# AlgoLab/rs-vgaligner

Hardware: AMD Instinct MI355X
Metric: aligned reads/sec (10 kbp ONT vs HLA graph) (higher is better)
Workload: dtype int32+f64

## Files before the change

include/vga_hip.h:

```cpp
#ifndef VGA_HIP_H
#define VGA_HIP_H

#include <stddef.h>
#include <stdint.h>

#ifdef __cplusplus
extern "C" {
#endif

#define VGA_OK 0
#define VGA_ERR_ARG (-1)
#define VGA_ERR_HIP (-2)
#define VGA_ERR_NOMEM (-3)
#define VGA_ERR_UNSUPPORTED (-4)
#define VGA_ERR_NO_INDEX (-5)
#define VGA_ERR_NO_DEVICE (-6)
#define VGA_ERR_POOL (-7)

#define VGA_NO_PRED (-1)

#define VGA_MAX_KMER_LENGTH 32

typedef struct vga_ctx vga_ctx;

// ... 106 lines not shown
    int32_t *best_score;
    uint64_t *path_off;
    uint32_t *abpoa_nodes;
    uint32_t *graph_nodes;
    uint32_t *aln_start_offset;
    uint32_t *aln_end_offset;
    uint32_t *n_aligned_bases;
    uint64_t *cigar_off;
    char *cigar;
    uint64_t *cs_off;
    char *cs;
    uint64_t *n_rows;
    uint64_t *n_cells;
    uint64_t *n_value_cells;
    float ms_dp, ms_traceback, ms_total;
} vga_poa_result;
void vga_poa_result_free(vga_poa_result *r);

int vga_poa_batch(vga_ctx *ctx, uint64_t n, const uint64_t *node_ptr, const uint64_t *node_off,
                  const char *nodes_concat, const uint64_t *edge_ptr, const uint32_t *edge_src,
                  const uint32_t *edge_dst, const uint64_t *query_off, const char *queries_concat,
                  const vga_poa_params *params, vga_poa_result **out);

typedef struct {
    uint64_t n_reads;
    uint8_t *aligned;
    uint64_t *path_off;
    uint64_t *path_handles;
    uint32_t *path_length;
    uint32_t *path_start;
    uint32_t *path_end;
    uint32_t *block_length;
    int32_t *best_score;
    uint64_t *cigar_off;
    char *cigar;
    uint64_t *cs_off;
    char *cs;
    uint64_t poa_rows, poa_cells, poa_value_cells, poa_problems;
    float ms_subgraph, ms_dp, ms_traceback, ms_total;
    uint64_t result_bytes;
} vga_align_result;

int vga_align_batch(vga_batch *b, const vga_map_result *chains, uint32_t align_best_n,
                    const vga_poa_params *params, vga_align_result **out);
void vga_align_result_free(vga_align_result *r);
int vga_align_prepare(vga_ctx *ctx, uint64_t n_reads, uint32_t max_read_len);

int vga_coverage_begin(vga_ctx *ctx);
int vga_coverage_read(vga_ctx *ctx, uint32_t *base_depth , uint32_t *node_reads ,
                      uint32_t *edge_reads , uint64_t *n_alignments);
int vga_coverage_reset(vga_ctx *ctx);
int vga_coverage_end(vga_ctx *ctx);

int vga_path_support_begin(vga_ctx *ctx, uint32_t n_paths, const uint64_t *step_off , const uint64_t *steps,
                           uint64_t *n_pairs_without_edge);
// ... 112 lines not shown
```

rs-vgaligner_amd/binding.py:

```python
from __future__ import annotations

import ctypes as C
import os
from typing import List, Optional, Sequence

import numpy as np

_HERE = os.path.dirname(os.path.abspath(__file__))
LIB_PATH = os.environ.get("VGA_LIB") or os.path.join(_HERE, "libvga_hip.so")

VGA_OK = 0
VGA_MAX_KMER_LENGTH = 32
VGA_STRANDS_FORWARD = 0
VGA_STRANDS_BOTH = 1
ERR_NAMES = {-1: "VGA_ERR_ARG", -2: "VGA_ERR_HIP", -3: "VGA_ERR_NOMEM", -4: "VGA_ERR_UNSUPPORTED",
             -5: "VGA_ERR_NO_INDEX", -6: "VGA_ERR_NO_DEVICE", -7: "VGA_ERR_POOL"}

PILEUP_COLUMNS = ("A", "C", "G", "T", "N", "del", "ins")

ABI_SYMBOLS = [
    "vga_ctx_create", "vga_ctx_destroy", "vga_last_error", "vga_ctx_synchronize", "vga_abi_version",
    "vga_index_upload", "vga_batch_create", "vga_batch_destroy", "vga_batch_strands", "vga_map_default_params", "vga_map_batch",
    "vga_map_result_free", "vga_poa_default_params", "vga_poa_result_free", "vga_poa_batch", "vga_align_batch",
    "vga_align_result_free", "vga_last_kernel_times", "vga_chain_paths_text", "vga_chain_text_free",
# ... 118 lines not shown
        ("max_chain_score", _P(C.c_double)), ("best_pred_id", _P(C.c_int32)), ("curr_max", _P(C.c_double)),
        ("n_chains", C.c_uint64), ("chain_off", _P(C.c_uint64)), ("chain_placeholder", _P(C.c_uint8)),
        ("chain_anchor_off", _P(C.c_uint64)), ("chain_anchor_idx", _P(C.c_uint32)),
        ("ms_probe", C.c_float), ("ms_sort", C.c_float), ("ms_chain", C.c_float), ("ms_total", C.c_float),
        ("n_hits", C.c_uint64), ("strand", _P(C.c_uint8)),
    ]


class PoaResult(C.Structure):
    _fields_ = [
        ("n", C.c_uint64), ("ok", _P(C.c_uint8)), ("best_score", _P(C.c_int32)), ("path_off", _P(C.c_uint64)),
        ("abpoa_nodes", _P(C.c_uint32)), ("graph_nodes", _P(C.c_uint32)), ("aln_start_offset", _P(C.c_uint32)),
        ("aln_end_offset", _P(C.c_uint32)), ("n_aligned_bases", _P(C.c_uint32)), ("cigar_off", _P(C.c_uint64)),
        ("cigar", _P(C.c_char)), ("cs_off", _P(C.c_uint64)), ("cs", _P(C.c_char)), ("n_rows", _P(C.c_uint64)),
        ("n_cells", _P(C.c_uint64)), ("n_value_cells", _P(C.c_uint64)), ("ms_dp", C.c_float), ("ms_traceback", C.c_float), ("ms_total", C.c_float),
    ]


class AlignResult(C.Structure):
    _fields_ = [
        ("n_reads", C.c_uint64), ("aligned", _P(C.c_uint8)), ("path_off", _P(C.c_uint64)), ("path_handles", _P(C.c_uint64)),
        ("path_length", _P(C.c_uint32)), ("path_start", _P(C.c_uint32)), ("path_end", _P(C.c_uint32)),
        ("block_length", _P(C.c_uint32)), ("best_score", _P(C.c_int32)), ("cigar_off", _P(C.c_uint64)),
        ("cigar", _P(C.c_char)), ("cs_off", _P(C.c_uint64)), ("cs", _P(C.c_char)),
        ("poa_rows", C.c_uint64), ("poa_cells", C.c_uint64), ("poa_value_cells", C.c_uint64), ("poa_problems", C.c_uint64),
        ("ms_subgraph", C.c_float), ("ms_dp", C.c_float), ("ms_traceback", C.c_float), ("ms_total", C.c_float),
        ("result_bytes", C.c_uint64),
    ]


class KernelTime(C.Structure):
    _fields_ = [("name", C.c_char_p), ("ms", C.c_float), ("launches", C.c_uint32), ("algorithmic_bytes", C.c_uint64),
                ("busy_ms", C.c_float), ("reserved", C.c_uint32)]


_lib = None


def load_library():
    global _lib
    if _lib is not None:
        return _lib
# ... 344 lines not shown
        tp = int(self.path_off[-1])
        self.abpoa_nodes = _np(r.abpoa_nodes, tp, np.uint32)
        self.graph_nodes = _np(r.graph_nodes, tp, np.uint32)
        self.aln_start_offset = _np(r.aln_start_offset, n, np.uint32)
        self.aln_end_offset = _np(r.aln_end_offset, n, np.uint32)
        self.n_aligned_bases = _np(r.n_aligned_bases, n, np.uint32)
        self.cigar_off = _np(r.cigar_off, n + 1, np.uint64)
        self.cs_off = _np(r.cs_off, n + 1, np.uint64)
        cig = C.string_at(r.cigar, int(self.cigar_off[-1])) if n else b""
        cs = C.string_at(r.cs, int(self.cs_off[-1])) if n else b""
        self.cigar = [cig[int(self.cigar_off[i]):int(self.cigar_off[i + 1]) - 1].decode() for i in range(n)]
        self.cs = [cs[int(self.cs_off[i]):int(self.cs_off[i + 1]) - 1].decode() for i in range(n)]
        self.n_rows = _np(r.n_rows, n, np.uint64)
        self.n_cells = _np(r.n_cells, n, np.uint64)
        self.n_value_cells = _np(r.n_value_cells, n, np.uint64)
        self.ms = {"dp": r.ms_dp, "traceback": r.ms_traceback, "total": r.ms_total}
        L.vga_poa_result_free(ptr)


class AlignOut:
    def __init__(self, L, ptr):
        r = ptr.contents
        R = int(r.n_reads)
        self.n_reads = R
        self.aligned = _np(r.aligned, R, np.uint8)
        self.path_off = _np(r.path_off, R + 1, np.uint64)
        self.path_handles = _np(r.path_handles, int(self.path_off[-1]), np.uint64)
        self.path_length = _np(r.path_length, R, np.uint32)
        self.path_start = _np(r.path_start, R, np.uint32)
        self.path_end = _np(r.path_end, R, np.uint32)
        self.block_length = _np(r.block_length, R, np.uint32)
        self.best_score = _np(r.best_score, R, np.int32)
        self.cigar_off = _np(r.cigar_off, R + 1, np.uint64)
        self.cs_off = _np(r.cs_off, R + 1, np.uint64)
        cig = C.string_at(r.cigar, int(self.cigar_off[-1])) if R else b""
        cs = C.string_at(r.cs, int(self.cs_off[-1])) if R else b""
        self.cigar = [cig[int(self.cigar_off[i]):int(self.cigar_off[i + 1]) - 1].decode() for i in range(R)]
        self.cs = [cs[int(self.cs_off[i]):int(self.cs_off[i + 1]) - 1].decode() for i in range(R)]
        self.poa_rows, self.poa_cells, self.poa_problems = int(r.poa_rows), int(r.poa_cells), int(r.poa_problems)
        self.poa_value_cells = int(r.poa_value_cells)
        self.ms = {"subgraph": r.ms_subgraph, "dp": r.ms_dp, "traceback": r.ms_traceback, "total": r.ms_total}
        L.vga_align_result_free(ptr)


class Batch:
    def __init__(self, ctx: "Context", seqs: Sequence):
        self.ctx = ctx
        L = ctx.L
        self.seqs = list(seqs)
        raw = [s if isinstance(s, (bytes, bytearray)) else s.encode() for s in self.seqs]
        self._concat = b"".join(raw)
        off = np.zeros(len(self.seqs) + 1, dtype=np.uint64)
        if self.seqs:
            off[1:] = np.cumsum([len(s) for s in raw], dtype=np.uint64)
        self._off = off
# ... 57 lines not shown
        t0 = _t.perf_counter()
        self.ctx._check(L.vga_map_batch(self.h, C.byref(mp), C.byref(m)))
        t1 = _t.perf_counter()
        kt_map = self.ctx.kernel_times()
        try:
            a = _P(AlignResult)()
            self.ctx._check(L.vga_align_batch(self.h, m, best_n, C.byref(pp), C.byref(a)))
            self.ctx._last_reads = len(self.seqs)
            t2 = _t.perf_counter()
            kt_aln = self.ctx.kernel_times()
            r, q = a.contents, m.contents
            R = int(r.n_reads)
            aligned = int(np.ctypeslib.as_array(r.aligned, shape=(R,)).sum()) if R else 0
            out = dict(n_reads=R, aligned=aligned, n_anchors=int(q.n_anchors), n_hits=int(q.n_hits),
                       poa_rows=int(r.poa_rows), poa_cells=int(r.poa_cells), poa_value_cells=int(r.poa_value_cells),
                       poa_problems=int(r.poa_problems), path_bases=int(np.ctypeslib.as_array(r.path_length, shape=(R,)).sum()) if R else 0,
                       cigar_bytes=int(r.cigar_off[R]) if R else 0, result_bytes=int(r.result_bytes),
                       ms_map=float(q.ms_total), ms_probe=float(q.ms_probe), ms_sort=float(q.ms_sort), ms_chain=float(q.ms_chain),
                       ms_align=float(r.ms_total), ms_subgraph=float(r.ms_subgraph), ms_dp_summed_launches=float(r.ms_dp),
                       ms_traceback=float(r.ms_traceback), kernels=kt_map + kt_aln)
            if on_results is not None:
                on_results(q, r)
            t3 = _t.perf_counter()
            L.vga_align_result_free(a)
        finally:
            L.vga_map_result_free(m)
        t4 = _t.perf_counter()
        out["ms_wall_map_call"] = (t1 - t0) * 1e3
        out["ms_wall_align_call"] = (t2 - t1) * 1e3
        out["ms_wall_free"] = (t4 - t3) * 1e3
        return out
# ... 529 lines not shown
```

rs-vgaligner_amd/csrc/vga_align.hip:

```cpp
#include "vga_align_plan.hpp"
#include "vga_common.hpp"
#include "vga_coverage.hpp"
#include "vga_path_edit.hpp"
#include "vga_path_support.hpp"
#include "vga_pileup.hpp"
#include "vga_insertion.hpp"
#include "vga_poa_internal.hpp"
#include "vga_subgraph_host.hpp"

#include <algorithm>
#include <atomic>
#include <chrono>
#include <memory>

extern "C" void vga_align_result_free(vga_align_result *r)
{
    if (!r) return;
    free(r->aligned); free(r->path_off); free(r->path_handles); free(r->path_length); free(r->path_start);
    free(r->path_end); free(r->block_length); free(r->best_score); free(r->cigar_off); free(r->cigar);
    free(r->cs_off); free(r->cs);
    free(r);
}

namespace {
// ... 272 lines not shown
        res->path_length[r] = it.n_path;
        res->path_start[r] = it.start_off;
        res->path_end[r] = it.end_off;
        res->block_length[r] = it.aligned;
        res->best_score[r] = it.score;
        if (it.cs_p) {
            memcpy(res->cigar + res->cigar_off[r], it.cigar_p, it.cigar_n); res->cigar[res->cigar_off[r] + it.cigar_n] = 0;
            memcpy(res->cs + res->cs_off[r], it.cs_p, it.cs_n); res->cs[res->cs_off[r] + it.cs_n] = 0;
        } else {
            memcpy(res->cigar + res->cigar_off[r], it.cigar.c_str(), it.cigar.size() + 1);
            memcpy(res->cs + res->cs_off[r], it.cs.c_str(), it.cs.size() + 1);
        }
    });
    res->poa_problems = n;
    for (uint64_t p = 0; p < n; p++) {
        res->poa_rows += items[p].n_rows; res->poa_cells += items[p].n_cells; res->poa_value_cells += items[p].n_vcells;
    }
    res->ms_subgraph = (float)sub_ms;
    res->ms_dp = tm.ms_dp;
    res->ms_traceback = tm.ms_tb;
    res->result_bytes = tm.result_bytes;
    res->ms_total = (float)std::chrono::duration<double, std::milli>(std::chrono::steady_clock::now() - t0).count();
    tr.mark("assemble records");
    if (tr.on && !on_device) sg_host_walk::trace_thread_time();
    return VGA_OK;
}

}

static int vga_align_batch_impl(vga_batch *b, const vga_map_result *m, uint32_t align_best_n, const vga_poa_params *params,
                               vga_align_result **out)
// ... 39 lines not shown
```

rs-vgaligner_amd/csrc/vga_poa_internal.hpp:

```cpp
#pragma once

#include <cstdint>
#include <functional>
#include <string>
#include <vector>

#include "vga_common.hpp"
#include "vga_subgraph.hpp"

struct poa_view {
    const uint64_t *node_off;
    const char *nodes;
    uint64_t n_nodes;
    const uint32_t *esrc, *edst;
    uint64_t n_edges;
    const char *query;
    uint32_t qlen;
};

struct poa_item {
    uint8_t ok = 0;
    int32_t score = 0;
    uint32_t start_off = 0, end_off = 0, aligned = 0;
    uint64_t n_rows = 0, n_cells = 0, n_vcells = 0;
    uint32_t n_path = 0;
    bool deduped = false;
    std::vector<uint32_t> rows;
    std::vector<uint32_t> gnodes;
    std::string cigar, cs;
    const char *cs_p = nullptr, *cigar_p = nullptr;
    const uint32_t *gnodes_p = nullptr;
    uint32_t cs_n = 0, cigar_n = 0, gnodes_n = 0;
};

struct poa_timing {
    float ms_dp = 0, ms_tb = 0, ms_total = 0;
    uint64_t result_bytes = 0;
};

// ... 16 lines not shown
```

rs-vgaligner_amd/csrc/vga_poa_launch.hpp:

```cpp
#pragma once

#include "vga_common.hpp"
#include "vga_poa_shape.hpp"
#include "vga_subgraph.hpp"

#define POA_CHUNK (1ull << 20)
#define POA_RING_SPAN 32
#define POA_SLOTS 4

#define POA_ST_OK 0
#define POA_ST_POOL 1
#define POA_ST_NOALN 2
#define POA_ST_TRACE 3
#define POA_ST_RETRY 5

struct poa_prob {
    uint64_t node0;
    uint64_t pred0;
    uint64_t sink0;
    uint64_t q0;
    uint64_t ops0;
    uint64_t row0;
    uint64_t seq0;
    uint32_t n_sink;
// ... 9 lines not shown
struct poa_row {
    int32_t beg, end;
    uint64_t doff, voff;
    int32_t lmax, rmax;
    uint32_t pred, npred;
    int32_t base, hmax;
};
static_assert(sizeof(poa_row) == 48 && offsetof(poa_row, pred) == 32, "poa_row layout");

struct poa_out {
    int32_t score;
    uint32_t row;
    int32_t status;
    uint32_t maxw;
    uint64_t cells, vcells;
    uint32_t nops, pad;
    uint64_t t_begin, t_end;
};

struct poa_dev_params {
    int32_t match, mismatch, o1, e1, o2, e2, banded;
};

#define POA_NIL 0xFFFFFFFFu
#define POA_LISTS 64
#define POA_LIST_STRIDE 16
struct poa_chunk_pool {
    unsigned long long *head;
    uint32_t *next;
    const uint64_t *seg_base;
    uint32_t cps_log2;
// ... 66 lines not shown
```

rs-vgaligner_amd/csrc/vga_poa_pool.hpp:

```cpp
#pragma once

#include <atomic>
#include <chrono>
#include <condition_variable>
#include <memory>
#include <mutex>
#include <thread>
#include <vector>

#include "vga_common.hpp"
#include "vga_poa_launch.hpp"

struct poa_slot {
    vga_dbuf<poa_prob> d_probs;
    vga_dbuf<uint4> d_ntab;
    vga_dbuf<uint32_t> d_seq32, d_preds, d_sink, d_orow, d_ids;
    vga_dbuf<uint8_t> d_ops;
    vga_dbuf<poa_row> d_rows;
    vga_dbuf<poa_out> d_outs;
    vga_dbuf<char> d_q;
    vga_hbuf<poa_prob> h_probs;
    vga_hbuf<uint4> h_ntab;
    vga_hbuf<uint32_t> h_seq32, h_preds, h_sink, h_ids;
    vga_hbuf<char> h_q;
    vga_dbuf<char> d_text;
    vga_dbuf<poa_text_out> d_touts;
    vga_dbuf<unsigned long long> d_tcur;
    struct out_set {
        vga_hbuf<uint32_t> h_orow;
        vga_hbuf<uint8_t> h_ops;
        vga_hbuf<char> h_seq;
        vga_hbuf<poa_out> h_outs;
        vga_hbuf<char> h_text;
        char *text_p = nullptr;
        vga_hbuf<poa_text_out> h_touts;
        vga_hbuf<unsigned long long> h_tcur;
        bool text = false;
        uint64_t tot_ops = 0, tot_seq = 0;
    } outs[2];
    uint32_t uses = 0;
};

#define POA_SEG_LOG2 32
#define POA_MAX_SEGS 80
struct poa_ws {
    poa_slot slot[POA_SLOTS];
    vga_dbuf<unsigned long long> d_next;
    vga_hbuf<unsigned long long> h_next;
    hipStream_t extra[POA_SLOTS] = {};
    double pool_scale = 1.35;
    struct seg_t { uint8_t *p; uint64_t size; };
    std::mutex mu;
// ... 178 lines not shown
```

rs-vgaligner_amd/csrc/vga_poa_run.hip:

```cpp
#include "vga_common.hpp"
#include "vga_oplist.hpp"
#include "vga_poa_internal.hpp"
#include "vga_poa_pool.hpp"

#include <algorithm>
#include <chrono>
#include <memory>
#include <thread>

namespace {

struct poa_prep {
    bool ok = false;
    uint32_t N = 0, qlen = 0;
    int32_t longest = 0;
    uint32_t life = 1;
    std::vector<uint4> ntab;
    std::vector<uint32_t> preds, sinks;
    std::vector<uint32_t> first_row;
    uint32_t n_ntab = 0, n_preds = 0, n_sinks = 0;
    const uint32_t *first_row_p = nullptr;
};

void poa_prepare(const poa_view &v, poa_prep &g, bool first_edge)
// ... 79 lines not shown
}

inline char lower(char c) { return (c >= 'A' && c <= 'Z') ? (char)(c + 32) : c; }

template <typename F>
void parallel_for(uint64_t n, F f) { vga_parallel_for(n, f); }

void poa_post_one(const poa_slot::out_set &S, uint64_t at, poa_item &it, const poa_prep &g, const poa_prob &pb, const poa_view &view, bool dev, bool keep_text)
{
    const poa_out &ho = S.h_outs.p[at];
    if (ho.status == POA_ST_POOL || ho.status == POA_ST_RETRY) return;
    it.ok = ho.status == POA_ST_OK ? 1 : 0;
    it.score = ho.score;
    it.n_cells = ho.cells;
    it.n_vcells = ho.vcells;
    if (!it.ok) return;
    if (S.text && S.h_touts.p[at].flags == 1u) {
        const poa_text_out &t = S.h_touts.p[at];
        const uint32_t *runs = (const uint32_t *)(S.text_p + t.runs_off);
        if (keep_text) {
            it.cs_p = S.text_p + t.cs_off; it.cs_n = t.cs_len;
            it.cigar_p = S.text_p + t.cg_off; it.cigar_n = t.cg_len;
            it.gnodes_p = runs; it.gnodes_n = t.n_runs;
            it.cs.clear(); it.cigar.clear(); it.gnodes.clear();
        } else {
            it.cs.assign(S.text_p + t.cs_off, t.cs_len);
            it.cigar.assign(S.text_p + t.cg_off, t.cg_len);
            it.gnodes.assign(runs, runs + t.n_runs);
        }
        it.rows.clear();
// ... 77 lines not shown
        it.end_off = it.rows.back() - frow[it.gnodes.back()] + 1;
    }
}

struct sub_t { uint64_t i0, i1; double raw_est; int slot; int oset; bool general = false; bool arena = false; };
struct range_t { uint64_t first, second; bool general; bool arena; };
struct launch_t {
    uint64_t i0 = 0, i1 = 0;
    int slot = 0, oset = 0;
    bool general = false, arena = false;
    uint32_t nb = 0;
    double raw_est = 0;
    uint64_t tot_nodes = 0, tot_preds = 0, tot_sink = 0, tot_q = 0, tot_ops = 0, tot_rows = 0, tot_seq = 0;
    bool text_on_device = false;
    bool fused = false;
    uint8_t *pool_base = nullptr;
    std::chrono::steady_clock::time_point t0;
};

struct poa_call {
    vga_ctx *const ctx;
    poa_feed &feed;
    const vga_poa_params *const params;
    std::vector<poa_item> &out;
    poa_timing &tm;
    const uint64_t n;
    std::vector<poa_view> &views;
    const poa_switches sw;
    const poa_family family;
    const std::chrono::steady_clock::time_point t_host0 = std::chrono::steady_clock::now();
// ... 355 lines not shown
        sum_w += estw[order[i]];
    }
    in.mean_w = sum_w / (double)L.nb;
    in.left = order.size() - L.i0;
    in.in_flight = in_flight_other;
    in.n_cu = (uint32_t)ctx->n_cu;
    in.giant = feed.klass && feed.klass[order[L.i0]];
    in.general = L.general;
    in.arena = L.arena;
    in.fused = L.fused = family != POA_FAM_LDS && sw.tb_fused;
    in.default_penalties = P.o1 == 4 && P.e1 == 2 && P.o2 == 24 && P.e2 == 1;
    in.family = family;
    any_fused = any_fused || L.fused;
    const poa_shape sh = poa_choose_shape(in, sw);
    trace_shape(L, sh, in.mean_w, in.max_w);
    L.pool_base = L.arena ? nullptr : W.classic + (uint64_t)L.slot * pool.half_pool;
    poa_chunk_pool cp_arg = pool.CP;
    if (!L.arena) cp_arg.n_slots = 0;
    const poa_t5_args a = {S.d_probs.p, S.d_q.p, S.d_ntab.p, S.d_seq32.p, S.d_preds.p, S.d_rows.p, L.pool_base, W.d_next.p + L.slot, pool.half_pool,
                           S.d_outs.p, (L.fused ? S.d_ops.p : nullptr), (L.fused ? S.d_orow.p : nullptr), cp_arg, sh.lds_cols, sh.hg_cols, sh.win_mask, P,
                           (in.giant && sw.giant_prio) ? 1u : 0u};
    chk(poa_launch_dp(ctx->device, st, sh, L.nb, a, S.d_sink.p));
    vga_timer_end(ctx, t_dp);
    const int t_tb = vga_timer_begin(ctx, "poa_traceback", 0, st);
    if (!L.fused) poa_launch_traceback(st, sh.kernel, L.nb, bufs_of(S), L.pool_base);
    vga_timer_end(ctx, t_tb);
}

void poa_call::enqueue_results(const launch_t &L)
{
    hipStream_t st = sarr[L.slot];
    poa_slot &S = W.slot[L.slot];
    poa_slot::out_set &O = S.outs[L.oset];
    const uint32_t nb = L.nb;
    chk(hipMemcpyAsync(O.h_outs.p, S.d_outs.p, nb * sizeof(poa_out), hipMemcpyDeviceToHost, st));
    chk(hipMemcpyAsync(W.h_next.p + L.slot, W.d_next.p + L.slot, sizeof(unsigned long long), hipMemcpyDeviceToHost, st));
    O.text = L.text_on_device;
    O.tot_ops = L.tot_ops; O.tot_seq = L.tot_seq;
    if (L.text_on_device) {
        uint64_t arena = std::min<uint64_t>(2ull * L.tot_ops + 64ull * nb + 4096ull, 0xF0000000ull);
        if (sw.has_text_arena) arena = std::min<uint64_t>(arena, sw.text_arena);
        chk(S.d_text.reserve(arena + 16)); chk(S.d_touts.reserve(nb)); chk(S.d_tcur.reserve(1));
        chk(O.h_touts.reserve(nb)); chk(O.h_tcur.reserve(1));
        if (launch_err == hipSuccess) {
            const int t_tx = vga_timer_begin(ctx, "poa_text", 0, st);
            chk(hipMemsetAsync(S.d_tcur.p, 0, sizeof(unsigned long long), st));
            chk(poa_launch_text(st, nb, bufs_of(S), S.d_text.p, (uint32_t)arena, S.d_tcur.p, S.d_touts.p));
            vga_timer_end(ctx, t_tx);
            chk(hipMemcpyAsync(O.h_touts.p, S.d_touts.p, nb * sizeof(poa_text_out), hipMemcpyDeviceToHost, st));
            chk(hipMemcpyAsync(O.h_tcur.p, S.d_tcur.p, sizeof(unsigned long long), hipMemcpyDeviceToHost, st));
        }
    } else {
// ... 363 lines not shown
    if (n_reads == 0 || max_read_len == 0 || max_read_len >= (1u << 24)) return VGA_OK;
    const poa_switches sw = poa_read_switches();
    if (sw.arenas_off) return VGA_OK;
    if (4ull * ((uint64_t)max_read_len + 8) > POA_CHUNK) return VGA_OK;
    if (hipSetDevice(ctx->device) != hipSuccess) return vga_set_error(ctx, VGA_ERR_HIP, "vga_align_prepare: hipSetDevice failed");
    vga_ctx_scope scope(ctx);
    poa_pool_prepare(ctx, sw, n_reads, max_read_len);
    return VGA_OK;
}

extern "C" void vga_poa_result_free(vga_poa_result *r)
{
    if (!r) return;
    free(r->ok); free(r->best_score); free(r->path_off); free(r->abpoa_nodes); free(r->graph_nodes);
    free(r->aln_start_offset); free(r->aln_end_offset); free(r->n_aligned_bases); free(r->cigar_off);
    free(r->cigar); free(r->cs_off); free(r->cs); free(r->n_rows); free(r->n_cells); free(r->n_value_cells);
    free(r);
}

static int vga_poa_batch_impl(vga_ctx *ctx, uint64_t n, const uint64_t *node_ptr, const uint64_t *node_off,
                             const char *nodes_concat, const uint64_t *edge_ptr, const uint32_t *edge_src,
                             const uint32_t *edge_dst, const uint64_t *query_off, const char *queries_concat,
                             const vga_poa_params *params, vga_poa_result **out)
{
    if (!ctx || !out || !params || (n && (!node_ptr || !node_off || !nodes_concat || !edge_ptr || !query_off || !queries_concat)))
        return VGA_ERR_ARG;
    *out = nullptr;
    (void)hipSetDevice(ctx->device);
    vga_ctx_scope scope(ctx);
    vga_release_deferred(ctx);
    poa_feed feed;
// ... 12 lines not shown
    vga_poa_result *res = (vga_poa_result *)calloc(1, sizeof(vga_poa_result));
    if (!res) return vga_set_error(ctx, VGA_ERR_NOMEM, "out of host memory (POA result)");
    auto nomem = [&]() { vga_poa_result_free(res); return vga_set_error(ctx, VGA_ERR_NOMEM, "out of host memory (POA result of %llu problems)", (unsigned long long)n); };
    res->n = n;
    res->ok = pmalloc<uint8_t>(n);
    res->best_score = pmalloc<int32_t>(n);
    res->path_off = pmalloc<uint64_t>(n + 1);
    res->aln_start_offset = pmalloc<uint32_t>(n);
    res->aln_end_offset = pmalloc<uint32_t>(n);
    res->n_aligned_bases = pmalloc<uint32_t>(n);
    res->cigar_off = pmalloc<uint64_t>(n + 1);
    res->cs_off = pmalloc<uint64_t>(n + 1);
    res->n_rows = pmalloc<uint64_t>(n);
    res->n_cells = pmalloc<uint64_t>(n);
    res->n_value_cells = pmalloc<uint64_t>(n);
    if (!res->ok || !res->best_score || !res->path_off || !res->aln_start_offset || !res->aln_end_offset || !res->n_aligned_bases ||
        !res->cigar_off || !res->cs_off || !res->n_rows || !res->n_cells || !res->n_value_cells)
        return nomem();
    uint64_t tp = 0, tc = 0, ts = 0;
    for (uint64_t p = 0; p < n; p++) {
        res->path_off[p] = tp; res->cigar_off[p] = tc; res->cs_off[p] = ts;
        tp += items[p].rows.size(); tc += items[p].cigar.size() + 1; ts += items[p].cs.size() + 1;
    }
    res->path_off[n] = tp; res->cigar_off[n] = tc; res->cs_off[n] = ts;
    res->abpoa_nodes = pmalloc<uint32_t>(tp);
    res->graph_nodes = pmalloc<uint32_t>(tp);
    res->cigar = pmalloc<char>(tc);
    res->cs = pmalloc<char>(ts);
    if (!res->abpoa_nodes || !res->graph_nodes || !res->cigar || !res->cs) return nomem();
    for (uint64_t p = 0; p < n; p++) {
        const poa_item &it = items[p];
        res->ok[p] = it.ok; res->best_score[p] = it.score; res->aln_start_offset[p] = it.start_off;
        res->aln_end_offset[p] = it.end_off; res->n_aligned_bases[p] = it.aligned; res->n_rows[p] = it.n_rows;
        res->n_cells[p] = it.n_cells; res->n_value_cells[p] = it.n_vcells;
        if (!it.rows.empty()) {
            memcpy(res->abpoa_nodes + res->path_off[p], it.rows.data(), it.rows.size() * 4);
            memcpy(res->graph_nodes + res->path_off[p], it.gnodes.data(), it.gnodes.size() * 4);
        }
        memcpy(res->cigar + res->cigar_off[p], it.cigar.c_str(), it.cigar.size() + 1);
        memcpy(res->cs + res->cs_off[p], it.cs.c_str(), it.cs.size() + 1);
    }
    res->ms_dp = tm.ms_dp;
    res->ms_traceback = tm.ms_tb;
    res->ms_total = tm.ms_total;
    *out = res;
    return VGA_OK;
}

extern "C" int vga_poa_batch(vga_ctx *ctx, uint64_t n, const uint64_t *node_ptr, const uint64_t *node_off,
// ... 13 lines not shown
```

rs-vgaligner_amd/csrc/vga_poa_t5.hpp:

```cpp
#pragma once

#include "vga_poa_row.hpp"

__device__ __forceinline__ uint64_t t5_uniform64(uint64_t v)
{
    return ((uint64_t)(uint32_t)__builtin_amdgcn_readfirstlane((int)(v >> 32)) << 32) | (uint32_t)__builtin_amdgcn_readfirstlane((int)(uint32_t)v);
}

#define POA_T5_ARGS_OFFSET 40
__device__ __forceinline__ const poa_t5_args *t5_kargs()
{
    uint32_t off = POA_T5_ARGS_OFFSET;
    asm volatile("" : "+s"(off));
    return (const poa_t5_args *)((const char *)__builtin_amdgcn_kernarg_segment_ptr() + off);
}
template <int NT, bool DEF>
__global__ __launch_bounds__(NT) __attribute__((amdgpu_waves_per_eu(5)))
void k_poa_dp_t5(const poa_prob *__restrict__ probs, const char *__restrict__ queries,
                                                       const uint4 *__restrict__ node_tab, const uint32_t *__restrict__ seq32,
                                                       const uint32_t *__restrict__ preds, const poa_t5_args A)
{
    poa_row *rows = A.rows;
    uint8_t *pool_arg = A.pool;
    const uint32_t lds_cols = t5_own(A.lds_cols), hg_cols = t5_own(A.hg_cols), win_mask = t5_own(A.win_mask);
    enum : uint32_t { ST_CHUNKED = 1u, ST_QPLAIN = 2u, ST_FAILED = 4u, ST_PREV_LDS = 8u, ST_PREV_FAR_USE = 16u };
    uint32_t st = (A.cp.n_slots != 0 ? ST_CHUNKED : 0u) | ST_PREV_LDS;
#define chunked ((st & ST_CHUNKED) != 0)
#define failed ((st & ST_FAILED) != 0)
#define q_plain ((st & ST_QPLAIN) != 0)
#define prev_lds ((st & ST_PREV_LDS) != 0)
#define prev_far_use ((st & ST_PREV_FAR_USE) != 0)
    struct { int match, mismatch, o1, e1, o2, e2, banded; } P = {t5_own(A.P.match), t5_own(A.P.mismatch), A.P.o1, A.P.e1, A.P.o2, A.P.e2, t5_own(A.P.banded)};
    constexpr int NW = NT / 64;
    constexpr int STEP = NT * 4;
    extern __shared__ __attribute__((aligned(16))) uint8_t smem[];
    int4 *sX = (int4 *)smem;
    int4 *sRed = sX + 2 * NW;
    int32_t *edgeW = (int32_t *)(sRed + NW);
    int32_t *sSink = edgeW + 4;
    uint64_t *sChunk = (uint64_t *)(sSink + 4);
    constexpr int HDR = (3 * NW + 1 + 1 + 2) * 16;
    int32_t *Hs = (int32_t *)(smem + HDR);
    uint16_t *Gs = (uint16_t *)(smem + HDR + 4ull * hg_cols);
    uint16_t *Qn = (uint16_t *)(smem + HDR + 6ull * hg_cols);
    const int edge_idx = (int)(edgeW - Hs);

// ... 116 lines not shown
            const uint64_t rb = (maxrow * (uint64_t)ring_rows + POA_CHUNK - 1) & ~(POA_CHUNK - 1);
            if (tid == 0) sChunk[2] = atomicAdd(A.pool_next, (unsigned long long)rb);
            __syncthreads();
            const uint64_t b = t5_uniform64(sChunk[2]);
            if (b + rb > A.pool_size || rb >= (1ull << 32)) st |= ST_FAILED;
            ring_base = b;
        }
    }
    if (tid == 0) { sSink[2] = POA_NEG; sSink[3] = 0; }
    int prev_beg = 0, prev_end = -1;
    uint32_t seq_word = 0, seq_word_idx = 0xFFFFFFFFu;

    for (uint32_t v = 0; v < n_nodes && !failed; v++) {
    const uint4 nt = ntab[v];
    const uint32_t nlen = nt.y & 0xFFFFFFu;
    for (uint32_t tn = 0; tn < nlen && !failed; tn++) {
        asm volatile("" : "+s"(st));
        POA_MARK("row_topo");
        const uint32_t r = nt.x + tn;
        const bool last = tn + 1 == nlen;
        const bool is_sink = last && (nt.z >> 31) != 0;
        const uint32_t ps = nt.w;
        uint32_t gb = 0;
        if (v > 0) {
            const uint32_t bi = r - 1;
            if ((bi & 3u) == 0 || (bi >> 2) != seq_word_idx) { seq_word_idx = bi >> 2; seq_word = seqw[seq_word_idx]; }
            gb = (seq_word >> (8u * (bi & 3u))) & 0xffu;
        }
        const bool simple = r > 0 && prev_lds && (tn > 0 || ((nt.y >> 24) == 1u && ps == r - 1));
        const bool writer = wv == (int)(r % (uint32_t)NW);
        POA_MARK("row_prevmax");
        int prev_lmax = 0, prev_rmax = 0;
        if (r > 0) {
            int4 rw = make_int4(INT32_MIN, INT32_MAX, INT32_MIN, 0);
            if (lane < NW) rw = sRed[lane];
            int b = rw.x, t;
            t = poa_dpp<0x111, 0xf>(INT32_MIN, b); b = t > b ? t : b;
            if (NW > 2) { t = poa_dpp<0x112, 0xf>(INT32_MIN, b); b = t > b ? t : b; }
            if (NW > 4) { t = poa_dpp<0x114, 0xf>(INT32_MIN, b); b = t > b ? t : b; }
            if (NW > 8) { t = poa_dpp<0x118, 0xf>(INT32_MIN, b); b = t > b ? t : b; }
            const int rbest = __builtin_amdgcn_readlane(b, NW - 1);
            const uint64_t tie = __builtin_amdgcn_ballot_w64(rw.x == rbest);
            if (__builtin_expect(__builtin_popcountll(tie) == 1, 1)) {
                const int w1 = __builtin_ctzll(tie);
                prev_lmax = __builtin_amdgcn_readlane(rw.y, w1);
// ... 16 lines not shown
                }
                prev_lmax = __builtin_amdgcn_readlane(lm, NW - 1);
                prev_rmax = __builtin_amdgcn_readlane(rm, NW - 1);
            }
            if (prev_far_use && writer && lane == 0) { R[r - 1].lmax = prev_lmax; R[r - 1].rmax = prev_rmax; }
        }
        POA_MARK("row_setup");
        const int remain = (int)(nt.z & 0x3fffffffu) + (int)(nlen - 1 - tn);
        int beg, end, np, pbeg = prev_beg, pend = prev_end;
        bool first, single, sp_near;
        uint32_t sp = r - 1;
        uint64_t vpo = 0;
        if (__builtin_expect(simple, 1)) {
            first = tn == 0;
            np = 1; single = true; sp_near = true;
            const int mpl = prev_lmax + 1, mpr = prev_rmax + 1;
            if (!P.banded) { beg = 0; end = qlen; }
            else {
                const int diag = qlen - remain;
                const int lo = mpl < diag ? mpl : diag;
                const int hi = mpr > diag ? mpr : diag;
                beg = lo - bw; if (beg < 0) beg = 0;
                end = hi + bw; if (end > qlen) end = qlen;
            }
        } else {
            first = tn == 0 && v > 0;
            np = v == 0 ? 0 : (tn == 0 ? (int)(nt.y >> 24) : 1);
            bool far = r > 0 && !prev_lds;
            if (first) {
                if (np == 1) far |= ps != r - 1;
                else
// ... 26 lines not shown
                const int lo = mpl < diag ? mpl : diag;
                const int hi = mpr > diag ? mpr : diag;
                beg = lo - bw; if (beg < 0) beg = 0;
                end = hi + bw; if (end > qlen) end = qlen;
            }
            if (single && !sp_near) {
                pbeg = __builtin_amdgcn_readfirstlane(R[sp].beg);
                pend = __builtin_amdgcn_readfirstlane(R[sp].end);
                vpo = t5_uniform64(R[sp].voff);
            }
        }
        const int bal = beg & ~3;
        const int W = (end - bal + 1 + 3) & ~3;
        const bool wide = (uint32_t)W + 8u > hg_cols;
        const bool keep = last || wide;
        const uint64_t doff = alloc(dcur, dend, (uint32_t)W * (np > 1 ? 4u : 1u), 0);
        uint64_t voff = 0;
        if (last && !failed) {
            if (r == 0 || (nt.z & 0x40000000u)) voff = chunked ? alloc(dcur, dend, 6u * (uint32_t)W, 0) : alloc(vcur, vendp, 6u * (uint32_t)W, 1);
            else {
                voff = ring_base + (uint64_t)ring_head * ((6u * (uint32_t)((qlen + 8) & ~3) + 15u) & ~15u);
                ring_head = ring_head + 1 == ring_rows ? 0 : ring_head + 1;
            }
        } else if (wide) voff = wide_scratch + (r & 1u) * 6ull * lds_cols;
        if (__builtin_expect(failed, 0)) break;
        if (writer && lane == 0) {
            uint32_t *rec = (uint32_t *)(R + r);
            *(uint4 *)rec = make_uint4((uint32_t)beg, (uint32_t)end, (uint32_t)doff, (uint32_t)(doff >> 32));
            *(uint2 *)(rec + 4) = make_uint2((uint32_t)voff, (uint32_t)(voff >> 32));
            *(HIP_vector_type<uint32_t, 3> *)(rec + 8) = HIP_vector_type<uint32_t, 3>(ps, first ? (uint32_t)np : 0u, keep ? 1u : 0u);
        }
        uint8_t *Vrow = pool + voff;
        uint8_t *drow = pool + doff;
        const uint32_t gd = gb - (uint32_t)'A';
        const bool acgt = gd < 20u && ((0x80045u >> gd) & 1u);
        const int sc_eq = acgt ? P.match : 0, sc_ne = acgt ? -P.mismatch : 0;
        const int gsh = (int)((gb >> 1) & 3u);
        const int ne4t = 4 * sc_ne + 1, mm4 = 4 * (sc_eq - sc_ne);
        const bool staged = !simple && r > 0 && !wide && q_plain;
        if (staged) {
            POA_MARK("row_stage");
            if (chunked) {
                bool no_row = false;
                for (int t = 0; t < np; t++) no_row |= t5_uniform64(R[np == 1 ? sp : plist[ps + t]].voff) == 0;
                if (__builtin_expect(no_row, 0)) st |= ST_FAILED;
// ... 73 lines not shown
                        *(uint32_t *)(drow + 2ull * W + c) = (uint32_t)a1[0] | ((uint32_t)a1[1] << 8) | ((uint32_t)a1[2] << 16) | ((uint32_t)a1[3] << 24);
                        *(uint32_t *)(drow + 3ull * W + c) = (uint32_t)a2[0] | ((uint32_t)a2[1] << 8) | ((uint32_t)a2[2] << 16) | ((uint32_t)a2[3] << 24);
                    }
                }
            }
            POA_LDS_BARRIER();
            pbeg = bal > 0 ? bal - 1 : 0;
            pend = bal + W - 1;
        }
        const uint8_t *Vp = pool + vpo;
        const int balp = pbeg & ~3;

        POA_MARK("row_steps");
        enum : uint32_t { F_SINGLE = 1u, F_NEAR = 2u, F_PLAIN = 4u, F_WIDE = 8u, F_KEEP = 16u, F_SINK = 32u, F_MULTI = 64u, F_SRC = 128u };
        const uint32_t rowf = (single ? F_SINGLE : 0u) | (sp_near ? F_NEAR : 0u) | (q_plain ? F_PLAIN : 0u) | (wide ? F_WIDE : 0u) |
                              (keep ? F_KEEP : 0u) | (is_sink ? F_SINK : 0u) | (np > 1 ? F_MULTI : 0u) | (r == 0 ? F_SRC : 0u);
        int best = INT32_MIN, lpos = beg, rpos = beg;
        const bool hot = (simple || staged) && !wide && q_plain;
        const int rlim = end < pend ? end : pend;
        auto run_steps = [&](auto hot_c) __attribute__((always_inline)) {
        constexpr bool HOT = decltype(hot_c)::value;
        int carry1 = POA_IDENT, carry2 = POA_IDENT, left1 = POA_IDENT, left2 = POA_IDENT;
        int next_left = 0;
        int buf = 0;
        for (int c0 = 0; c0 < W; c0 += STEP, buf ^= 1) {
            uint32_t f = HOT ? (rowf & (F_KEEP | F_SINK)) : rowf;
            asm volatile("" : "+s"(f));
            if (HOT) f |= F_SINGLE | F_NEAR | F_PLAIN;
            const int c = c0 + 4 * tid;
            const int j0 = bal + c;
            const bool lane_act = j0 <= end;
            const int jw0 = bal + c0 + 256 * wv, jw1 = jw0 + 255;
            const bool wave_act = jw0 <= end;
            int d_lp = jw0 - beg, d_rp = rlim - jw1, d_lq = (jw0 > beg ? jw0 : beg) - pbeg - 1;
            asm volatile("" : "+s"(d_lp), "+s"(d_rp), "+s"(d_lq));
            const uint32_t e_lp = (uint32_t)d_lp >> 31;
            const uint32_t e_rp = (uint32_t)d_rp >> 31;
            const uint32_t e_lq = (uint32_t)d_lq >> 31;
            const bool lp = e_lp != 0, rp = e_rp != 0, lq = e_lq != 0;
            int htt[4], ht4[4], e1t[4], e2t[4], pmeta[4];
            int agg1 = POA_IDENT, agg2 = POA_IDENT, alast1 = POA_IDENT, alast2 = POA_IDENT;
// ... 330 lines not shown
                                const int kf = hb[0] == m4 ? 0 : (hb[1] == m4 ? 1 : (hb[2] == m4 ? 2 : 3));
                                const int kl = hb[3] == m4 ? 3 : (hb[2] == m4 ? 2 : (hb[1] == m4 ? 1 : 0));
                                if (m4 > best) { best = m4; lpos = j0 + kf; }
                                rpos = j0 + kl;
                            }
                        }
                        if (__builtin_expect((f & F_SINK) != 0, 0)) {
                            const int kq = qlen - j0;
#pragma unroll
                            for (int k = 0; k < 4; k++)
                                if (kq == k) sSink[0] = h4[k];
                        }
                        if (!EDGE || j0 <= end) {
                            const int4 hq = make_int4(h4[0], h4[1], h4[2], h4[3]);
                            const uint2 gq = make_uint2((uint32_t)ga, (uint32_t)gbb);
                            if (!(f & F_WIDE)) {
                                *(int4 *)(Hs + (j0 & win_mask)) = hq;
                                *(uint2 *)(Gs + (j0 & win_mask)) = gq;
                            }
                            *(uint32_t *)(drow + c) = (uint32_t)dirq;
                            if (f & F_KEEP) {
                                *(int4 *)((int32_t *)Vrow + c) = hq;
                                *(uint2 *)(Vrow + 4ll * W + 2ll * c) = gq;
                            }
                        }
                    };
                    if (__builtin_expect((e_lp | e_rp) != 0, 0)) phase2(std::true_type{});
                    else phase2(std::false_type{});
        if constexpr (HOT) POA_MARK("hot_p2_slow"); else POA_MARK("p2_slow");
                } else if (lane_act) {
                    int beg_ = beg, end_ = end;
// ... 66 lines not shown
                if (mine) { red[0] = best; red[1] = lpos; red[2] = rpos; }
            } else {
                int lm = mine ? lpos : INT32_MAX, rm = mine ? rpos : INT32_MIN;
                lm = poa_wave_scan_min(lm);
                rm = poa_wave_scan_max(rm);
                if (lane == 63) { red[0] = wb; red[1] = lm; red[2] = rm; }
            }
        }
        POA_LDS_BARRIER();
        POA_MARK("row_end");
        if (__builtin_expect(is_sink, 0) && tid == 0) {
            const int val = (qlen >= beg && qlen <= end) ? sSink[0] >> 2 : POA_NEG;
            if (sSink[3] == 0 || val > sSink[2]) { sSink[2] = val; sSink[3] = (int)r + 1; }
        }
        prev_beg = beg; prev_end = end;
        st = (st & ~(ST_PREV_LDS | ST_PREV_FAR_USE)) | (wide ? 0u : ST_PREV_LDS) | (last ? ST_PREV_FAR_USE : 0u);
    }
    }
    POA_MARK("epilogue");
    __syncthreads();
    if (tid >= 64) return;
    const poa_t5_args E = *t5_kargs();
    const poa_prob pe = E.probs[blockIdx.x];
    poa_out &O = E.outs[blockIdx.x];
    int status = POA_ST_OK;
    uint32_t start_row = 0;
    int sink_best = POA_NEG;
    if (failed) status = POA_ST_POOL;
    else {
        sink_best = __builtin_amdgcn_readfirstlane(sSink[2]);
        const int sr = __builtin_amdgcn_readfirstlane(sSink[3]);
        start_row = sr ? (uint32_t)(sr - 1) : 0u;
        status = (sr != 0 && sink_best > POA_NEG / 2) ? POA_ST_OK : POA_ST_NOALN;
        const poa_row *Rr = E.rows + pe.row0;
        uint64_t cells = 0, vcells = 0;
        int maxw = 0;
        for (uint32_t r = (uint32_t)lane; r <= pe.N; r += 64) {
            const int b = Rr[r].beg, e = Rr[r].end, kp = Rr[r].base;
            const int W = (e - (b & ~3) + 1 + 3) & ~3;
            maxw = W > maxw ? W : maxw;
            if (r > 0) cells += (uint64_t)(e - b + 1);
            if (kp) vcells += (uint64_t)(e - b + 1);
        }
        for (int sh = 32; sh > 0; sh >>= 1) {
            cells += __shfl_down(cells, sh);
            vcells += __shfl_down(vcells, sh);
            const int m2 = __shfl_down(maxw, sh);
            maxw = m2 > maxw ? m2 : maxw;
        }
        if (tid == 0) { O.cells = cells; O.vcells = vcells; O.maxw = (uint32_t)maxw; }
    }
    if (tid == 0) {
        if (failed) { O.cells = 0; O.vcells = 0; O.maxw = 0; }
        O.score = failed ? POA_NEG : sink_best;
        O.row = start_row;
        O.status = status;
    }
    if (E.tb_ops) {
        uint8_t *pool_e = E.cp.n_slots ? nullptr : E.pool;
        poa_traceback_wave<2>(*(tb_lds *)(smem + HDR), tid, pe, E.rows, E.preds, pool_e, O, E.tb_ops, E.tb_orow, 0, status, start_row);
    }
    if (tid == 0) {
        O.t_end = __builtin_amdgcn_s_memrealtime();
        if (E.cp.n_slots) {
            const uint32_t state_slot = (uint32_t)sSink[1];
            if (own_head != POA_NIL) poa_chunk_push(E.cp, blockIdx.x, own_head, (uint32_t)sChunk[3]);
            const uint64_t state_lo = (uint64_t)E.cp.state_base + (uint64_t)state_slot * E.cp.state_size;
            (void)atomicAdd(E.pool_next, (unsigned long long)own_chunks * POA_CHUNK + (vcur - state_lo));
            __builtin_amdgcn_fence(__ATOMIC_RELEASE, "agent");
            (void)atomicExch(&E.cp.slot_flag[state_slot], 0u);
        }
    }
}
#undef chunked
#undef failed
#undef q_plain
#undef prev_lds
#undef prev_far_use
```

Before: 10660.

## Skip LDS window writes for single-base held rows in the T5 POA kernel

Adds a 'hold' mode to the T5 POA DP kernel. When a single-base node is followed by a node whose only predecessor is the row before it, that row's H/G values are not written to the LDS window. The next row instead reads its band bounds from the global row record after a block barrier. The goal is to cut LDS store traffic for chains of single-base nodes, at the cost of an extra __syncthreads and global reads on the rows that follow. It also records held-row counts through the result structs and Python bindings.

```diff
diff --git a/include/vga_hip.h b/include/vga_hip.h
--- a/include/vga_hip.h
+++ b/include/vga_hip.h
@@ -144,6 +144,7 @@
     uint64_t *n_cells;
     uint64_t *n_value_cells;
     float ms_dp, ms_traceback, ms_total;
+    uint64_t *n_held_rows;
 } vga_poa_result;
 void vga_poa_result_free(vga_poa_result *r);
 
@@ -169,6 +170,7 @@
     uint64_t poa_rows, poa_cells, poa_value_cells, poa_problems;
     float ms_subgraph, ms_dp, ms_traceback, ms_total;
     uint64_t result_bytes;
+    uint64_t poa_held_rows;
 } vga_align_result;
 
 int vga_align_batch(vga_batch *b, const vga_map_result *chains, uint32_t align_best_n,
diff --git a/rs-vgaligner_amd/binding.py b/rs-vgaligner_amd/binding.py
--- a/rs-vgaligner_amd/binding.py
+++ b/rs-vgaligner_amd/binding.py
@@ -156,6 +156,7 @@
         ("aln_end_offset", _P(C.c_uint32)), ("n_aligned_bases", _P(C.c_uint32)), ("cigar_off", _P(C.c_uint64)),
         ("cigar", _P(C.c_char)), ("cs_off", _P(C.c_uint64)), ("cs", _P(C.c_char)), ("n_rows", _P(C.c_uint64)),
         ("n_cells", _P(C.c_uint64)), ("n_value_cells", _P(C.c_uint64)), ("ms_dp", C.c_float), ("ms_traceback", C.c_float), ("ms_total", C.c_float),
+        ("n_held_rows", _P(C.c_uint64)),
     ]
 
 
@@ -167,7 +168,7 @@
         ("cigar", _P(C.c_char)), ("cs_off", _P(C.c_uint64)), ("cs", _P(C.c_char)),
         ("poa_rows", C.c_uint64), ("poa_cells", C.c_uint64), ("poa_value_cells", C.c_uint64), ("poa_problems", C.c_uint64),
         ("ms_subgraph", C.c_float), ("ms_dp", C.c_float), ("ms_traceback", C.c_float), ("ms_total", C.c_float),
-        ("result_bytes", C.c_uint64),
+        ("result_bytes", C.c_uint64), ("poa_held_rows", C.c_uint64),
     ]
 
 
@@ -542,6 +543,7 @@
         self.n_rows = _np(r.n_rows, n, np.uint64)
         self.n_cells = _np(r.n_cells, n, np.uint64)
         self.n_value_cells = _np(r.n_value_cells, n, np.uint64)
+        self.n_held_rows = _np(r.n_held_rows, n, np.uint64)
         self.ms = {"dp": r.ms_dp, "traceback": r.ms_traceback, "total": r.ms_total}
         L.vga_poa_result_free(ptr)
 
@@ -567,6 +569,7 @@
         self.cs = [cs[int(self.cs_off[i]):int(self.cs_off[i + 1]) - 1].decode() for i in range(R)]
         self.poa_rows, self.poa_cells, self.poa_problems = int(r.poa_rows), int(r.poa_cells), int(r.poa_problems)
         self.poa_value_cells = int(r.poa_value_cells)
+        self.poa_held_rows = int(r.poa_held_rows)
         self.ms = {"subgraph": r.ms_subgraph, "dp": r.ms_dp, "traceback": r.ms_traceback, "total": r.ms_total}
         L.vga_align_result_free(ptr)
 
@@ -654,7 +657,7 @@
             aligned = int(np.ctypeslib.as_array(r.aligned, shape=(R,)).sum()) if R else 0
             out = dict(n_reads=R, aligned=aligned, n_anchors=int(q.n_anchors), n_hits=int(q.n_hits),
                        poa_rows=int(r.poa_rows), poa_cells=int(r.poa_cells), poa_value_cells=int(r.poa_value_cells),
-                       poa_problems=int(r.poa_problems), path_bases=int(np.ctypeslib.as_array(r.path_length, shape=(R,)).sum()) if R else 0,
+                       poa_held_rows=int(r.poa_held_rows), poa_problems=int(r.poa_problems), path_bases=int(np.ctypeslib.as_array(r.path_length, shape=(R,)).sum()) if R else 0,
                        cigar_bytes=int(r.cigar_off[R]) if R else 0, result_bytes=int(r.result_bytes),
                        ms_map=float(q.ms_total), ms_probe=float(q.ms_probe), ms_sort=float(q.ms_sort), ms_chain=float(q.ms_chain),
                        ms_align=float(r.ms_total), ms_subgraph=float(r.ms_subgraph), ms_dp_summed_launches=float(r.ms_dp),
diff --git a/rs-vgaligner_amd/csrc/vga_align.hip b/rs-vgaligner_amd/csrc/vga_align.hip
--- a/rs-vgaligner_amd/csrc/vga_align.hip
+++ b/rs-vgaligner_amd/csrc/vga_align.hip
@@ -310,7 +310,7 @@
     });
     res->poa_problems = n;
     for (uint64_t p = 0; p < n; p++) {
-        res->poa_rows += items[p].n_rows; res->poa_cells += items[p].n_cells; res->poa_value_cells += items[p].n_vcells;
+        res->poa_rows += items[p].n_rows; res->poa_cells += items[p].n_cells; res->poa_value_cells += items[p].n_vcells; res->poa_held_rows += items[p].n_hold;
     }
     res->ms_subgraph = (float)sub_ms;
     res->ms_dp = tm.ms_dp;
diff --git a/rs-vgaligner_amd/csrc/vga_poa_internal.hpp b/rs-vgaligner_amd/csrc/vga_poa_internal.hpp
--- a/rs-vgaligner_amd/csrc/vga_poa_internal.hpp
+++ b/rs-vgaligner_amd/csrc/vga_poa_internal.hpp
@@ -23,6 +23,7 @@
     int32_t score = 0;
     uint32_t start_off = 0, end_off = 0, aligned = 0;
     uint64_t n_rows = 0, n_cells = 0, n_vcells = 0;
+    uint64_t n_hold = 0;
     uint32_t n_path = 0;
     bool deduped = false;
     std::vector<uint32_t> rows;
diff --git a/rs-vgaligner_amd/csrc/vga_poa_launch.hpp b/rs-vgaligner_amd/csrc/vga_poa_launch.hpp
--- a/rs-vgaligner_amd/csrc/vga_poa_launch.hpp
+++ b/rs-vgaligner_amd/csrc/vga_poa_launch.hpp
@@ -47,7 +47,8 @@
     int32_t status;
     uint32_t maxw;
     uint64_t cells, vcells;
-    uint32_t nops, pad;
+    uint32_t nops;
+    uint32_t n_hold;
     uint64_t t_begin, t_end;
 };
 
diff --git a/rs-vgaligner_amd/csrc/vga_poa_pool.hpp b/rs-vgaligner_amd/csrc/vga_poa_pool.hpp
--- a/rs-vgaligner_amd/csrc/vga_poa_pool.hpp
+++ b/rs-vgaligner_amd/csrc/vga_poa_pool.hpp
@@ -36,6 +36,7 @@
         vga_hbuf<poa_text_out> h_touts;
         vga_hbuf<unsigned long long> h_tcur;
         bool text = false;
+        bool t5 = false;
         uint64_t tot_ops = 0, tot_seq = 0;
     } outs[2];
     uint32_t uses = 0;
diff --git a/rs-vgaligner_amd/csrc/vga_poa_run.hip b/rs-vgaligner_amd/csrc/vga_poa_run.hip
--- a/rs-vgaligner_amd/csrc/vga_poa_run.hip
+++ b/rs-vgaligner_amd/csrc/vga_poa_run.hip
@@ -117,6 +117,7 @@
     it.score = ho.score;
     it.n_cells = ho.cells;
     it.n_vcells = ho.vcells;
+    it.n_hold = S.t5 ? ho.n_hold : 0;
     if (!it.ok) return;
     if (S.text && S.h_touts.p[at].flags == 1u) {
         const poa_text_out &t = S.h_touts.p[at];
@@ -224,6 +225,7 @@
     uint64_t tot_nodes = 0, tot_preds = 0, tot_sink = 0, tot_q = 0, tot_ops = 0, tot_rows = 0, tot_seq = 0;
     bool text_on_device = false;
     bool fused = false;
+    bool t5 = false;
     uint8_t *pool_base = nullptr;
     std::chrono::steady_clock::time_point t0;
 };
@@ -609,6 +611,7 @@
     any_fused = any_fused || L.fused;
     const poa_shape sh = poa_choose_shape(in, sw);
     trace_shape(L, sh, in.mean_w, in.max_w);
+    L.t5 = sh.kernel == POA_K_T5;
     L.pool_base = L.arena ? nullptr : W.classic + (uint64_t)L.slot * pool.half_pool;
     poa_chunk_pool cp_arg = pool.CP;
     if (!L.arena) cp_arg.n_slots = 0;
@@ -631,6 +634,7 @@
     chk(hipMemcpyAsync(O.h_outs.p, S.d_outs.p, nb * sizeof(poa_out), hipMemcpyDeviceToHost, st));
     chk(hipMemcpyAsync(W.h_next.p + L.slot, W.d_next.p + L.slot, sizeof(unsigned long long), hipMemcpyDeviceToHost, st));
     O.text = L.text_on_device;
+    O.t5 = L.t5;
     O.tot_ops = L.tot_ops; O.tot_seq = L.tot_seq;
     if (L.text_on_device) {
         uint64_t arena = std::min<uint64_t>(2ull * L.tot_ops + 64ull * nb + 4096ull, 0xF0000000ull);
@@ -1024,7 +1028,7 @@
     if (!r) return;
     free(r->ok); free(r->best_score); free(r->path_off); free(r->abpoa_nodes); free(r->graph_nodes);
     free(r->aln_start_offset); free(r->aln_end_offset); free(r->n_aligned_bases); free(r->cigar_off);
-    free(r->cigar); free(r->cs_off); free(r->cs); free(r->n_rows); free(r->n_cells); free(r->n_value_cells);
+    free(r->cigar); free(r->cs_off); free(r->cs); free(r->n_rows); free(r->n_cells); free(r->n_value_cells); free(r->n_held_rows);
     free(r);
 }
 
@@ -1067,8 +1071,9 @@
     res->n_rows = pmalloc<uint64_t>(n);
     res->n_cells = pmalloc<uint64_t>(n);
     res->n_value_cells = pmalloc<uint64_t>(n);
+    res->n_held_rows = pmalloc<uint64_t>(n);
     if (!res->ok || !res->best_score || !res->path_off || !res->aln_start_offset || !res->aln_end_offset || !res->n_aligned_bases ||
-        !res->cigar_off || !res->cs_off || !res->n_rows || !res->n_cells || !res->n_value_cells)
+        !res->cigar_off || !res->cs_off || !res->n_rows || !res->n_cells || !res->n_value_cells || !res->n_held_rows)
         return nomem();
     uint64_t tp = 0, tc = 0, ts = 0;
     for (uint64_t p = 0; p < n; p++) {
@@ -1085,7 +1090,7 @@
         const poa_item &it = items[p];
         res->ok[p] = it.ok; res->best_score[p] = it.score; res->aln_start_offset[p] = it.start_off;
         res->aln_end_offset[p] = it.end_off; res->n_aligned_bases[p] = it.aligned; res->n_rows[p] = it.n_rows;
-        res->n_cells[p] = it.n_cells; res->n_value_cells[p] = it.n_vcells;
+        res->n_cells[p] = it.n_cells; res->n_value_cells[p] = it.n_vcells; res->n_held_rows[p] = it.n_hold;
         if (!it.rows.empty()) {
             memcpy(res->abpoa_nodes + res->path_off[p], it.rows.data(), it.rows.size() * 4);
             memcpy(res->graph_nodes + res->path_off[p], it.gnodes.data(), it.gnodes.size() * 4);
diff --git a/rs-vgaligner_amd/csrc/vga_poa_t5.hpp b/rs-vgaligner_amd/csrc/vga_poa_t5.hpp
--- a/rs-vgaligner_amd/csrc/vga_poa_t5.hpp
+++ b/rs-vgaligner_amd/csrc/vga_poa_t5.hpp
@@ -23,13 +23,16 @@
     poa_row *rows = A.rows;
     uint8_t *pool_arg = A.pool;
     const uint32_t lds_cols = t5_own(A.lds_cols), hg_cols = t5_own(A.hg_cols), win_mask = t5_own(A.win_mask);
-    enum : uint32_t { ST_CHUNKED = 1u, ST_QPLAIN = 2u, ST_FAILED = 4u, ST_PREV_LDS = 8u, ST_PREV_FAR_USE = 16u };
+    enum : uint32_t { ST_CHUNKED = 1u, ST_QPLAIN = 2u, ST_FAILED = 4u, ST_PREV_LDS = 8u, ST_PREV_FAR_USE = 16u, ST_HELD = 32u, ST_HOLD_CAND = 64u };
+    enum : uint32_t { F_HOLD = 256u };
+    static_assert(F_HOLD >> 3 == ST_HELD && ST_HOLD_CAND << 2 == F_HOLD, "the hold bits become one another by a shift");
     uint32_t st = (A.cp.n_slots != 0 ? ST_CHUNKED : 0u) | ST_PREV_LDS;
 #define chunked ((st & ST_CHUNKED) != 0)
 #define failed ((st & ST_FAILED) != 0)
 #define q_plain ((st & ST_QPLAIN) != 0)
 #define prev_lds ((st & ST_PREV_LDS) != 0)
 #define prev_far_use ((st & ST_PREV_FAR_USE) != 0)
+#define prev_held ((st & ST_HELD) != 0)
     struct { int match, mismatch, o1, e1, o2, e2, banded; } P = {t5_own(A.P.match), t5_own(A.P.mismatch), A.P.o1, A.P.e1, A.P.o2, A.P.e2, t5_own(A.P.banded)};
     constexpr int NW = NT / 64;
     constexpr int STEP = NT * 4;
@@ -176,6 +179,13 @@
     for (uint32_t v = 0; v < n_nodes && !failed; v++) {
     const uint4 nt = ntab[v];
     const uint32_t nlen = nt.y & 0xFFFFFFu;
+    {
+        const uint4 nx = ntab[v + 1 < n_nodes ? v + 1 : v];
+        const uint32_t lrow = prev_held ? nt.w : nt.x - 1;
+        const bool simple0 = nt.x > 0 && prev_lds && (prev_held || ((nt.y >> 24) == 1u && nt.w == nt.x - 1));
+        const bool cand = nlen == 1u && v + 1 < n_nodes && simple0 && q_plain && (nx.y >> 24) == 1u && nx.w == lrow;
+        st = (st & ~ST_HOLD_CAND) | (cand ? ST_HOLD_CAND : 0u);
+    }
     for (uint32_t tn = 0; tn < nlen && !failed; tn++) {
         asm volatile("" : "+s"(st));
         POA_MARK("row_topo");
@@ -189,8 +199,10 @@
             if ((bi & 3u) == 0 || (bi >> 2) != seq_word_idx) { seq_word_idx = bi >> 2; seq_word = seqw[seq_word_idx]; }
             gb = (seq_word >> (8u * (bi & 3u))) & 0xffu;
         }
-        const bool simple = r > 0 && prev_lds && (tn > 0 || ((nt.y >> 24) == 1u && ps == r - 1));
+        const bool simple = r > 0 && prev_lds && (tn > 0 || prev_held || ((nt.y >> 24) == 1u && ps == r - 1));
         const bool writer = wv == (int)(r % (uint32_t)NW);
+        uint32_t holdf = (st & ST_HOLD_CAND) << 2;
+        asm volatile("" : "+s"(holdf));
         POA_MARK("row_prevmax");
         int prev_lmax = 0, prev_rmax = 0;
         if (r > 0) {
@@ -237,7 +249,14 @@
         if (__builtin_expect(simple, 1)) {
             first = tn == 0;
             np = 1; single = true; sp_near = true;
-            const int mpl = prev_lmax + 1, mpr = prev_rmax + 1;
+            int mpl = prev_lmax + 1, mpr = prev_rmax + 1;
+            if (__builtin_expect(prev_held, 0)) {
+                __syncthreads();
+                mpl = __builtin_amdgcn_readfirstlane(R[ps].lmax) + 1;
+                mpr = __builtin_amdgcn_readfirstlane(R[ps].rmax) + 1;
+                pbeg = __builtin_amdgcn_readfirstlane(R[ps].beg);
+                pend = __builtin_amdgcn_readfirstlane(R[ps].end);
+            }
             if (!P.banded) { beg = 0; end = qlen; }
             else {
                 const int diag = qlen - remain;
@@ -294,6 +313,7 @@
         const int W = (end - bal + 1 + 3) & ~3;
         const bool wide = (uint32_t)W + 8u > hg_cols;
         const bool keep = last || wide;
+        if (wide) holdf = 0;
         const uint64_t doff = alloc(dcur, dend, (uint32_t)W * (np > 1 ? 4u : 1u), 0);
         uint64_t voff = 0;
         if (last && !failed) {
@@ -308,7 +328,7 @@
             uint32_t *rec = (uint32_t *)(R + r);
             *(uint4 *)rec = make_uint4((uint32_t)beg, (uint32_t)end, (uint32_t)doff, (uint32_t)(doff >> 32));
             *(uint2 *)(rec + 4) = make_uint2((uint32_t)voff, (uint32_t)(voff >> 32));
-            *(HIP_vector_type<uint32_t, 3> *)(rec + 8) = HIP_vector_type<uint32_t, 3>(ps, first ? (uint32_t)np : 0u, keep ? 1u : 0u);
+            *(HIP_vector_type<uint32_t, 3> *)(rec + 8) = HIP_vector_type<uint32_t, 3>(ps, first ? (uint32_t)np : 0u, (keep ? 1u : 0u) | (holdf >> 7));
         }
         uint8_t *Vrow = pool + voff;
         uint8_t *drow = pool + doff;
@@ -412,7 +432,7 @@
         POA_MARK("row_steps");
         enum : uint32_t { F_SINGLE = 1u, F_NEAR = 2u, F_PLAIN = 4u, F_WIDE = 8u, F_KEEP = 16u, F_SINK = 32u, F_MULTI = 64u, F_SRC = 128u };
         const uint32_t rowf = (single ? F_SINGLE : 0u) | (sp_near ? F_NEAR : 0u) | (q_plain ? F_PLAIN : 0u) | (wide ? F_WIDE : 0u) |
-                              (keep ? F_KEEP : 0u) | (is_sink ? F_SINK : 0u) | (np > 1 ? F_MULTI : 0u) | (r == 0 ? F_SRC : 0u);
+                              (keep ? F_KEEP : 0u) | (is_sink ? F_SINK : 0u) | (np > 1 ? F_MULTI : 0u) | (r == 0 ? F_SRC : 0u) | holdf;
         int best = INT32_MIN, lpos = beg, rpos = beg;
         const bool hot = (simple || staged) && !wide && q_plain;
         const int rlim = end < pend ? end : pend;
@@ -422,7 +442,7 @@
         int next_left = 0;
         int buf = 0;
         for (int c0 = 0; c0 < W; c0 += STEP, buf ^= 1) {
-            uint32_t f = HOT ? (rowf & (F_KEEP | F_SINK)) : rowf;
+            uint32_t f = HOT ? (rowf & (F_KEEP | F_SINK | F_HOLD)) : rowf;
             asm volatile("" : "+s"(f));
             if (HOT) f |= F_SINGLE | F_NEAR | F_PLAIN;
             const int c = c0 + 4 * tid;
@@ -783,7 +803,7 @@
                         if (!EDGE || j0 <= end) {
                             const int4 hq = make_int4(h4[0], h4[1], h4[2], h4[3]);
                             const uint2 gq = make_uint2((uint32_t)ga, (uint32_t)gbb);
-                            if (!(f & F_WIDE)) {
+                            if (!(f & (HOT ? (uint32_t)F_HOLD : (uint32_t)F_WIDE))) {
                                 *(int4 *)(Hs + (j0 & win_mask)) = hq;
                                 *(uint2 *)(Gs + (j0 & win_mask)) = gq;
                             }
@@ -880,7 +900,7 @@
             if (sSink[3] == 0 || val > sSink[2]) { sSink[2] = val; sSink[3] = (int)r + 1; }
         }
         prev_beg = beg; prev_end = end;
-        st = (st & ~(ST_PREV_LDS | ST_PREV_FAR_USE)) | (wide ? 0u : ST_PREV_LDS) | (last ? ST_PREV_FAR_USE : 0u);
+        st = (st & ~(ST_PREV_LDS | ST_PREV_FAR_USE | ST_HELD)) | (wide ? 0u : ST_PREV_LDS) | (last ? ST_PREV_FAR_USE : 0u) | ((rowf & F_HOLD) >> 3);
     }
     }
     POA_MARK("epilogue");
@@ -901,23 +921,26 @@
         const poa_row *Rr = E.rows + pe.row0;
         uint64_t cells = 0, vcells = 0;
         int maxw = 0;
+        uint32_t n_hold = 0;
         for (uint32_t r = (uint32_t)lane; r <= pe.N; r += 64) {
             const int b = Rr[r].beg, e = Rr[r].end, kp = Rr[r].base;
             const int W = (e - (b & ~3) + 1 + 3) & ~3;
             maxw = W > maxw ? W : maxw;
             if (r > 0) cells += (uint64_t)(e - b + 1);
-            if (kp) vcells += (uint64_t)(e - b + 1);
+            if (kp & 1) vcells += (uint64_t)(e - b + 1);
+            n_hold += (uint32_t)(kp >> 1) & 1u;
         }
         for (int sh = 32; sh > 0; sh >>= 1) {
             cells += __shfl_down(cells, sh);
             vcells += __shfl_down(vcells, sh);
+            n_hold += __shfl_down(n_hold, sh);
             const int m2 = __shfl_down(maxw, sh);
             maxw = m2 > maxw ? m2 : maxw;
         }
-        if (tid == 0) { O.cells = cells; O.vcells = vcells; O.maxw = (uint32_t)maxw; }
+        if (tid == 0) { O.cells = cells; O.vcells = vcells; O.maxw = (uint32_t)maxw; O.n_hold = n_hold; }
     }
     if (tid == 0) {
-        if (failed) { O.cells = 0; O.vcells = 0; O.maxw = 0; }
+        if (failed) { O.cells = 0; O.vcells = 0; O.maxw = 0; O.n_hold = 0; }
         O.score = failed ? POA_NEG : sink_best;
         O.row = start_row;
         O.status = status;
@@ -943,3 +966,4 @@
 #undef q_plain
 #undef prev_lds
 #undef prev_far_use
+#undef prev_held
```

After: 10560. No clear change (-0.9%).
